# Animesh005/Torus-FHE

Measured on AMD Instinct MI355X. Metric: bootstrapped gates/sec (NAND, N=1024), higher is better.
Workload: dtype f64

## Files before the change

torus-fhe_amd/csrc/thfhe_sk.hip:

```cpp
#include <hip/hip_runtime.h>

#include <algorithm>
#include <cstdlib>
#include <memory>
#include <mutex>
#include <new>
#include <string>
#include <vector>

#include "../../include/thfhe_hip.h"
#include "thfhe_common.h"
#include "thfhe_dag.h"
#include "thfhe_devctx.h"
#include "thfhe_keyswitch.h"
#include "thfhe_lane.h"
#include "thfhe_pack.h"

using namespace thfhe;

namespace {

#include "thfhe_transform.h"

struct Lin {
    int32_t cb, cx, cy;
    int ysel;
};
__host__ __device__ inline bool gate_lin(int op, int which, Lin &L) {
    const int32_t E8 = 1 << 29, E4 = 1 << 30;
    switch (op) {
    case THFHE_NAND: L = Lin{E8, -1, -1, 1}; return true;
    case THFHE_OR: L = Lin{E8, 1, 1, 1}; return true;
    case THFHE_AND: L = Lin{-E8, 1, 1, 1}; return true;
    case THFHE_XOR: L = Lin{E4, 2, 2, 1}; return true;
    case THFHE_XNOR: L = Lin{-E4, -2, -2, 1}; return true;
    case THFHE_NOR: L = Lin{-E8, -1, -1, 1}; return true;
    case THFHE_ANDNY: L = Lin{-E8, -1, 1, 1}; return true;
    case THFHE_ANDYN: L = Lin{-E8, 1, -1, 1}; return true;
    case THFHE_ORNY: L = Lin{E8, -1, 1, 1}; return true;
    case THFHE_ORYN: L = Lin{E8, 1, -1, 1}; return true;
    case THFHE_MUX: L = which == 0 ? Lin{-E8, 1, 1, 1} : Lin{-E8, -1, 1, 2}; return true;
    case kOpIdentity: L = Lin{0, 1, 0, 1}; return true;
    default: return false;
    }
}

__global__ __launch_bounds__(256) void sk_prologue_kernel(const int32_t *__restrict__ in0, const int32_t *__restrict__ in1,
                                                           const int32_t *__restrict__ in2, int op, const int32_t *__restrict__ ops,
                                                           int rot_per_gate, int n, int n_pad, int log2_2n, long jobs,
                                                           int32_t *__restrict__ bara, int32_t *__restrict__ barb) {
    const long job = blockIdx.y;
    const int i = blockIdx.x * 256 + threadIdx.x;
    if (job >= jobs || i > n) return;
    const long gate = job / rot_per_gate;
    const int which = (int)(job % rot_per_gate);
    Lin L;
    gate_lin(ops ? ops[gate] : op, which, L);
    const size_t off = (size_t)gate * (n + 1) + i;
    uint32_t v = (uint32_t)L.cx * (uint32_t)in0[off];
    if (L.cy != 0) v += (uint32_t)L.cy * (uint32_t)(L.ysel == 2 ? in2[off] : in1[off]);
    if (i == n) {
        v += (uint32_t)L.cb;
        barb[job] = modswitch2n((int32_t)v, log2_2n);
    } else {
        bara[job * n_pad + i] = modswitch2n((int32_t)v, log2_2n);
    }
}

THFHE_STAMP_STORAGE

struct BRArgs {
    const cplx *bk;
    const cplx *tw;
    const int32_t *bara;
    const int32_t *barb;
    int32_t *out;
    long jobs;
    int n, n_pad, Bgbit;
    int32_t mu;
    const int32_t *tv;
    const int32_t *lut_idx;
    int theta;
    const int32_t *tv_a;
    const int32_t *mv_w;
    int mv_p, mv_box;
};

constexpr int kGate = 0, kLut = 1, kLutEnc = 2, kLutMv = 3;

#ifndef THFHE_RING_NF
#define THFHE_RING_NF 16
#endif
#ifndef THFHE_RING_LEAN_ROOTS
#define THFHE_RING_LEAN_ROOTS 1
#endif
#ifndef THFHE_RING_READ_FIRST
#define THFHE_RING_READ_FIRST 0
#endif
template <int L, int V = 5, int W = 8, int LUT = kGate>
__global__ __launch_bounds__(64 * W, W == 8 ? 2 : 1) void sk_blind_rotate_ring_kernel(BRArgs a) {
    __shared__ __attribute__((aligned(4096))) int32_t sAcc[W][2048];
    __shared__ cplx sX[W][kXbufSlots];
    __shared__ cplx sRing[3][512];
    constexpr int ROWS = 2 * L;
    constexpr int DPC = 8 / W;
    const int wave = __builtin_amdgcn_readfirstlane(threadIdx.x >> 6);
    const int lane = threadIdx.x & 63;
    const W64 w64{a.tw[TwRing1k::T2 + 1 * 8 + (lane & 7)]};
    const LaneRoots roots{a.tw[TwRing1k::ROOTS + 2 * lane], a.tw[TwRing1k::ROOTS + 2 * lane + 1]};
    const LaneTw tw = make_lane_tw(roots);
    LaneRootsF rootsf{a.tw[TwRing1k::ROOTSF + 2 * lane], a.tw[TwRing1k::ROOTSF + 2 * lane + 1]};
    W64 w64f = w64;
    LaneRoots rootsi = roots;
    const long job = (long)blockIdx.x * W + wave;
    const bool has_job = job < a.jobs;
    int32_t *acc = sAcc[wave];
    cplx *xb = sX[wave];
    const uniform_i32_ptr bara = as_uniform(a.bara + (has_job ? job : 0) * a.n_pad);
    const int Bgbit = a.Bgbit;
    if (has_job) {
        if constexpr (LUT == kLutEnc) {
            const size_t t = a.lut_idx ? (size_t)a.lut_idx[job] * 1024 : 0;
            acc_init_tlwe16(lane, acc, acc + 1024, a.barb[job], a.tv_a + t, a.tv + t);
        } else if constexpr (LUT == kLutMv) acc_init_tv16(lane, acc, acc + 1024, a.barb[job], a.tv);
        else if constexpr (LUT) acc_init_tv16(lane, acc, acc + 1024, a.barb[job], a.tv + (a.lut_idx ? (size_t)a.lut_idx[job] * 1024 : 0));
        else acc_init16(lane, acc, acc + 1024, a.barb[job], a.mu);
    }

    const long total_chunks = (long)a.n * ROWS * 4;
    const cplx *gsrc = a.bk + wave * (64 * DPC) + lane;
    long q_issue = 0;
    int slot_issue = 0;
    const uint32_t ring_base = (uint32_t)(size_t)(__attribute__((address_space(3))) void *)&sRing[0][0] + (uint32_t)wave * (1024u * DPC);
    auto issue = [&]() {
#pragma unroll
        for (int d = 0; d < DPC; d++) ring_dma(gsrc + 64 * d, ring_base + (uint32_t)slot_issue * 8192u + 1024u * d);
        if (q_issue + 1 < total_chunks) {
            gsrc += 512;
            q_issue++;
        }
        slot_issue = slot_issue == 2 ? 0 : slot_issue + 1;
    };
    __syncthreads();
    issue();
    issue();
    issue();
    int slot_use = 0;
    STAMP_DECL;

    for (int i = 0; i < a.n; i++) {
        const int ai = bara[i];
        const bool active = has_job && ai != 0;
        const int a2n = ai & 2047;
        cplx S[2][2][8];
#pragma unroll
        for (int c = 0; c < 2; c++)
#pragma unroll
            for (int h = 0; h < 2; h++)
#pragma unroll
                for (int m = 0; m < 8; m++) S[c][h][m] = cplx{0.0, 0.0};
        constexpr int NF = THFHE_RING_NF;
        uint32_t fld[NF];
#pragma unroll
        for (int r = 0; r < ROWS; r++) {
            cplx z[8];
            if (active) {
                int a2n_r = a2n;
                asm volatile("" : "+s"(a2n_r));
                if (r % L == 0) rotated_fields_keep<NF, W == 4>(lane, acc + (r / L) * 1024, a2n_r, L, Bgbit, fld);
                asm volatile("" : "+s"(a2n_r));
                mixed_digits_z<NF>(lane, acc + (r / L) * 1024, a2n_r, (r % L) + 1, L, Bgbit, fld, z);
                if (V & 4) {
                    if (THFHE_RING_LEAN_ROOTS && W == 8) opaque_in_place(rootsf.s), opaque_in_place(rootsf.w);
                    wave_fft_fwd_f(lane, z, xb, rootsf);
                } else if (!(V & 1)) wave_fft_fwd_r(lane, z, xb, roots, w64);
                else if (THFHE_RING_LEAN_ROOTS && W == 8) wave_fft_fwd_q(lane, z, xb, LaneRoots{opaque_cplx(roots.b), opaque_cplx(roots.s)}, w64);
                else wave_fft_fwd_q(lane, z, xb, tw, w64);
            }
            STAMP(0);
            cplx bA[4], bB[4];
#pragma unroll
            for (int c4 = 0; c4 < 4; c4++) {
                if (c4 == 0) ring_barrier<2 * DPC>(); else ring_barrier<DPC>();
                STAMP(1);
                const cplx *B = &sRing[slot_use][0];
#if THFHE_RING_READ_FIRST
                if (active) {
#pragma unroll
                    for (int m = 0; m < 4; m++) bA[m] = B[m * 64 + lane];
                }
                __builtin_amdgcn_sched_barrier(0);
                if (c4 > 0) issue();
                if (active) {
#else
                if (c4 > 0) issue();
                if (active) {
#pragma unroll
                    for (int m = 0; m < 4; m++) bA[m] = B[m * 64 + lane];
#endif
                    if (c4 > 0) {
#pragma unroll
                        for (int m = 0; m < 4; m++) cfma(S[(c4 - 1) >> 1][(c4 - 1) & 1][4 + m], z[4 + m], bB[m]);
                    }
#pragma unroll
                    for (int m = 0; m < 4; m++) bB[m] = B[(4 + m) * 64 + lane];
#pragma unroll
                    for (int m = 0; m < 4; m++) cfma(S[c4 >> 1][c4 & 1][m], z[m], bA[m]);
                }
                slot_use = slot_use == 2 ? 0 : slot_use + 1;
                STAMP(2);
            }
            ring_barrier<2 * DPC>();
            issue();
            STAMP(1);
            if (active) {
#pragma unroll
                for (int m = 0; m < 4; m++) cfma(S[1][1][4 + m], z[4 + m], bB[m]);
            }
            STAMP(2);
        }
        if (active) {
            wave_sync();
            cplx bc[4];
            if (V & 4) {
                if (THFHE_RING_LEAN_ROOTS && W == 8) opaque_in_place(rootsi.b);
                make_untwist_f(rootsi.b, bc);
            }
#pragma unroll
            for (int c = 0; c < 2; c++) {
                if (V & 4) {
                    wave_fft_inv_f<THFHE_RING_LEAN_ROOTS && W == 8>(lane, S[c][0], xb, w64f, rootsi, bc);
                    wave_fft_inv_f<THFHE_RING_LEAN_ROOTS && W == 8>(lane, S[c][1], xb, w64f, rootsi, bc);
                } else if ((V & 1) && !(V & 2)) {
                    if (THFHE_RING_LEAN_ROOTS && W == 8) {
                        wave_fft_inv_q(lane, S[c][0], xb, LaneRoots{opaque_cplx(roots.b), opaque_cplx(roots.s)}, w64);
                        wave_fft_inv_q(lane, S[c][1], xb, LaneRoots{opaque_cplx(roots.b), opaque_cplx(roots.s)}, w64);
                    } else {
                        wave_fft_inv_q(lane, S[c][0], xb, tw, w64);
                        wave_fft_inv_q(lane, S[c][1], xb, tw, w64);
                    }
                } else {
                    wave_fft_inv_r(lane, S[c][0], xb, roots, w64);
                    wave_fft_inv_r(lane, S[c][1], xb, roots, w64);
                }
                acc_update16(lane, acc + c * 1024, S[c][0], S[c][1]);
            }
            wave_sync();
        }
        STAMP(3);
    }
    STAMP_FLUSH(blockIdx.x, wave);
    asm volatile("s_waitcnt vmcnt(0)" ::: "memory");
    if (has_job) {
        if constexpr (LUT == kLutMv) {
            const uniform_i32_ptr w = as_uniform(a.mv_w) + (size_t)(a.lut_idx ? as_uniform(a.lut_idx)[job] : 0) * a.theta * a.mv_p;
            for (int j = 0; j < a.theta; j++) extract_mv16(lane, acc, acc + 1024, w + j * a.mv_p, a.mv_p, a.mv_box, a.out + (job * a.theta + j) * 1025);
        } else if constexpr (LUT) {
            for (int j = 0; j < a.theta; j++) extract_at16(lane, acc, acc + 1024, j, a.out + (job * a.theta + j) * 1025);
        } else {
            extract16(lane, acc, acc + 1024, a.out + job * 1025);
        }
    }
}

__device__ __forceinline__ void wg_barrier() { asm volatile("s_waitcnt lgkmcnt(0)\n\ts_barrier" ::: "memory"); }
__device__ __forceinline__ void pin() { asm volatile("" ::: "memory"); }

template <int L, int PACE = 1, int LUT = kGate>
__global__ __launch_bounds__(512, 2) void sk_blind_rotate_coop_kernel(BRArgs a) {
    constexpr int ROWS = 2 * L;
    __shared__ __attribute__((aligned(4096))) int32_t sAcc[2048];
    __shared__ cplx sSpec[ROWS][512];
    __shared__ cplx sX[8][kXbufSlots];
    const int wave = __builtin_amdgcn_readfirstlane(threadIdx.x >> 6);
    const int lane = threadIdx.x & 63;
    const W64 w64{a.tw[TwRing1k::T2 + 1 * 8 + (lane & 7)]};
    const LaneRoots roots{a.tw[TwRing1k::ROOTS + 2 * lane], a.tw[TwRing1k::ROOTS + 2 * lane + 1]};
    const long job = blockIdx.x;
    const uniform_i32_ptr bara = as_uniform(a.bara + job * a.n_pad);
    const int Bgbit = a.Bgbit;
    if (wave == 0) {
        if constexpr (LUT == kLutEnc) {
            const size_t t = a.lut_idx ? (size_t)a.lut_idx[job] * 1024 : 0;
            acc_init_tlwe16(lane, sAcc, sAcc + 1024, a.barb[job], a.tv_a + t, a.tv + t);
        } else if constexpr (LUT == kLutMv) acc_init_tv16(lane, sAcc, sAcc + 1024, a.barb[job], a.tv);
        else if constexpr (LUT) acc_init_tv16(lane, sAcc, sAcc + 1024, a.barb[job], a.tv + (a.lut_idx ? (size_t)a.lut_idx[job] * 1024 : 0));
        else acc_init16(lane, sAcc, sAcc + 1024, a.barb[job], a.mu);
    }
    const int c = (wave >> 1) & 1, h = wave & 1, half = wave >> 2, r0 = half * L;
    unsigned int *ap = reinterpret_cast<unsigned int *>(sAcc) + c * 1024;
    cplx *xb = sX[wave];

    int i = 0;
    while (i < a.n && bara[i] == 0) i++;
    cplx B[L][8];
    if (i < a.n) {
#pragma unroll
        for (int r = 0; r < L; r++) load8(lane, B[r], a.bk + bk_spec_index(i, r0 + r, c, h, ROWS));
    }
    wg_barrier();
    STAMP_DECL;
    while (i < a.n) {
        const int a2n = bara[i] & 2047;
        int inext = i + 1;
        while (inext < a.n && bara[inext] == 0) inext++;
        const int inl = inext < a.n ? inext : i;
        if (wave < ROWS) {
            cplx z[8];
            rotated_digits_z(lane, sAcc + (wave / L) * 1024, a2n, (wave % L) + 1, L, Bgbit, z);
            wave_fft_fwd_q(lane, z, xb, roots, w64);
#pragma unroll
            for (int m = 0; m < 8; m++) sSpec[wave][m * 64 + lane] = z[m];
        }
        STAMP(0);
        wg_barrier();
        STAMP(1);
        cplx S[8];
#pragma unroll
        for (int m = 0; m < 8; m++) S[m] = cplx{0.0, 0.0};
#pragma unroll
        for (int r = 0; r < L; r++) {
            cplx z[8];
#pragma unroll
            for (int m = 0; m < 8; m++) z[m] = sSpec[r0 + r][m * 64 + lane];
            mac8r(S, z, B[r]);
            pin();
        }
        STAMP(2);
        if (half == 1) {
#pragma unroll
            for (int m = 0; m < 8; m++) xb[m * 64 + lane] = S[m];
            pin();
            STAMP(3);
            wg_barrier();
            STAMP(4);
#pragma unroll
            for (int r = 0; r < L; r++) {
                const cplx *src = a.bk + bk_spec_index(inl, r0 + r, c, h, ROWS);
#pragma unroll
                for (int m = 0; m < 8; m++) {
                    B[r][m] = src[m * 64 + lane];
                    pin();
                    __builtin_amdgcn_s_sleep(PACE);
                }
            }
        } else {
            load8(lane, B[0], a.bk + bk_spec_index(inl, r0, c, h, ROWS));
            pin();
            STAMP(3);
            wg_barrier();
            STAMP(4);
            const cplx *px = sX[wave + 4];
#pragma unroll
            for (int m = 0; m < 8; m++) {
                const cplx v = px[m * 64 + lane];
                S[m].re += v.re;
                S[m].im += v.im;
            }
            wave_sync();
            invr_seg1(lane, S, xb, w64);
            pin();
            if (L > 1) load8(lane, B[L > 1 ? 1 : 0], a.bk + bk_spec_index(inl, r0 + 1, c, h, ROWS));
            pin();
            wave_sync();
            inv_seg2_ld(lane, S, xb);
            dft8<-1>(S);
            pin();
            if (L > 2) load8(lane, B[L > 2 ? 2 : 0], a.bk + bk_spec_index(inl, r0 + 2, c, h, ROWS));
            if (L > 3) load8(lane, B[L > 3 ? 3 : 0], a.bk + bk_spec_index(inl, r0 + 3, c, h, ROWS));
            pin();
            wave_transpose_hi3(S);
            invq_seg3(S, roots);
#pragma unroll
            for (int m = 0; m < 8; m++) {
                const int q = lane + 64 * m;
                atomicAdd(ap + q, round_lo32(S[m].re) << (16 * h));
                atomicAdd(ap + q + 512, round_lo32(S[m].im) << (16 * h));
            }
        }
        STAMP(3);
        wg_barrier();
        STAMP(5);
        i = inext;
    }
    STAMP_FLUSH(blockIdx.x, wave);
    if constexpr (LUT == kLutMv) {
        const uniform_i32_ptr w = as_uniform(a.mv_w) + (size_t)(a.lut_idx ? as_uniform(a.lut_idx)[job] : 0) * a.theta * a.mv_p;
        for (int j = wave; j < a.theta; j += 8)
            extract_mv16(lane, sAcc, sAcc + 1024, w + j * a.mv_p, a.mv_p, a.mv_box, a.out + (job * a.theta + j) * 1025);
    } else if constexpr (LUT) {
        if (wave < a.theta) extract_at16(lane, sAcc, sAcc + 1024, wave, a.out + (job * a.theta + wave) * 1025);
    } else {
        if (wave == 0) extract16(lane, sAcc, sAcc + 1024, a.out + job * 1025);
    }
}

__global__ __launch_bounds__(256) void sk_linear_kernel(const int32_t *__restrict__ in0, int32_t *__restrict__ out, size_t words, int negate) {
    const size_t q = (size_t)blockIdx.x * 256 + threadIdx.x;
    if (q < words) out[q] = negate ? (int32_t)(0u - (uint32_t)in0[q]) : in0[q];
}

}

struct THFHE_INTERNAL thfhe_ctx : DevCtx {
    thfhe_params p;
    int rec_words() const { return p.n + 1; }
    DevBuf d_bk;
    KsKey ksk;
    int coop_max_jobs = 768;
    int ring4_max_jobs = 1024;
    int n_pad = 0;
    DevBuf d_bara, d_barb, d_u;
    DevBuf d_tv, d_lut_idx;
    DevBuf d_tva;
    DevBuf d_mv_w;
    DevBuf d_tree_tab, d_tree_lwe, d_tree_a, d_tree_b;
    DevBuf d_dag_enc_a, d_dag_enc_b, d_dag_tv1;
    DevBuf d_dag_mv_tv0, d_dag_mv_w;
    DevBuf d_dag_lhe_tab_a, d_dag_lhe_tab_b, d_dag_lhe_fin_a, d_dag_lhe_fin_b, d_dag_lhe_words;
    DevBuf d_lhe_a, d_lhe_b, d_lhe_in[4];
    DevBuf d_wfa_tab;
    DevBuf d_sc_tab, d_sc_idx;
    int cus = 0;
    int wfa_chunk = 0;
    size_t tree_slice = 65536;
    Stage stage;
    DagBuffers dag;
    size_t dag_slice = 28672;
    hipEvent_t grp_ev[2] = {nullptr, nullptr};
    bool grp_valid = false;
    ~thfhe_ctx() {
        for (hipEvent_t e : grp_ev)
            if (e) (void)hipEventDestroy(e);
    }
};

struct THFHE_INTERNAL thfhe_tgsw_set {
    thfhe_ctx *ctx = nullptr;
    DevBuf spec;
    size_t count = 0;
    int d = 0;
};

namespace {

constexpr int kMaxEncLuts = 1 << 18;

int ensure_workspace(thfhe_ctx *c, size_t jobs) {
    int rc = c->d_bara.grow(jobs * c->n_pad * sizeof(int32_t));
    if (!rc) rc = c->d_barb.grow(jobs * sizeof(int32_t));
    if (!rc) rc = c->d_u.grow(jobs * 1025 * sizeof(int32_t));
    return rc;
}

template <int L, int LUT>
void launch_coop(const BRArgs &a, hipStream_t s) {
#ifdef THFHE_VARIANTS
    static const int pace = std::getenv("THFHE_COOP_PACE") ? std::atoi(std::getenv("THFHE_COOP_PACE")) : 1;
    if (!LUT && pace == 0) { hipLaunchKernelGGL((sk_blind_rotate_coop_kernel<L, 0>), dim3((unsigned)a.jobs), dim3(512), 0, s, a); return; }
    if (!LUT && pace == 2) { hipLaunchKernelGGL((sk_blind_rotate_coop_kernel<L, 2>), dim3((unsigned)a.jobs), dim3(512), 0, s, a); return; }
    if (!LUT && pace == 4) { hipLaunchKernelGGL((sk_blind_rotate_coop_kernel<L, 4>), dim3((unsigned)a.jobs), dim3(512), 0, s, a); return; }
#endif
    hipLaunchKernelGGL((sk_blind_rotate_coop_kernel<L, 1, LUT>), dim3((unsigned)a.jobs), dim3(512), 0, s, a);
}
template <int L, int LUT>
void launch_ring4(const BRArgs &a, hipStream_t s) {
    hipLaunchKernelGGL((sk_blind_rotate_ring_kernel<L, 5, 4, LUT>), dim3((unsigned)((a.jobs + 3) / 4)), dim3(256), 0, s, a);
}
template <int L, int LUT>
void launch_ring8(const BRArgs &a, hipStream_t s) {
    const dim3 grid((unsigned)((a.jobs + 7) / 8)), block(512);
#ifdef THFHE_VARIANTS
    static const int variant = std::getenv("THFHE_RING_VARIANT") ? std::atoi(std::getenv("THFHE_RING_VARIANT")) : 0;
    if (!LUT && variant == 8) { hipLaunchKernelGGL((sk_blind_rotate_ring_kernel<L, 0>), grid, block, 0, s, a); return; }
    if (!LUT && variant == 1) { hipLaunchKernelGGL((sk_blind_rotate_ring_kernel<L, 1>), grid, block, 0, s, a); return; }
    if (!LUT && variant == 3) { hipLaunchKernelGGL((sk_blind_rotate_ring_kernel<L, 3>), grid, block, 0, s, a); return; }
#endif
    hipLaunchKernelGGL((sk_blind_rotate_ring_kernel<L, 5, 8, LUT>), grid, block, 0, s, a);
}

template <int L, int LUT>
void launch_br(const BRArgs &a, hipStream_t s, int coop_max, int ring4_max) {
    auto piece = [&](long first, long count) {
        BRArgs b = a;
        b.bara += first * a.n_pad, b.barb += first, b.jobs = count;
        b.out += first * (LUT ? a.theta : 1) * 1025;
        if (LUT && b.lut_idx) b.lut_idx += first;
        return b;
    };
    constexpr long kRound = 2048;
    const long full = (coop_max > 0 || ring4_max > 0) ? a.jobs / kRound * kRound : a.jobs;
    if (full > 0) launch_ring8<L, LUT>(piece(0, full), s);
    const long r = a.jobs - full;
    if (r == 0) return;
    if (r <= coop_max) launch_coop<L, LUT>(piece(full, r), s);
    else if (r <= ring4_max) launch_ring4<L, LUT>(piece(full, r), s);
    else if (ring4_max > 0 && coop_max > 0 && r <= ring4_max + (coop_max < 256 ? coop_max : 256)) {
        launch_ring4<L, LUT>(piece(full, ring4_max), s);
        launch_coop<L, LUT>(piece(full + ring4_max, r - ring4_max), s);
    } else launch_ring8<L, LUT>(piece(full, r), s);
}

template <int LUT>
int launch_rotations(thfhe_ctx *c, const BRArgs &a) {
    switch (c->p.l) {
    case 1: launch_br<1, LUT>(a, c->stream, c->coop_max_jobs, c->ring4_max_jobs); break;
    case 2: launch_br<2, LUT>(a, c->stream, c->coop_max_jobs, c->ring4_max_jobs); break;
    case 3: launch_br<3, LUT>(a, c->stream, c->coop_max_jobs, c->ring4_max_jobs); break;
    case 4: launch_br<4, LUT>(a, c->stream, c->coop_max_jobs, c->ring4_max_jobs); break;
    default: return thfhe_fail(THFHE_E_UNSUPPORTED, "decomposition length l must be 1..4");
    }
    return THFHE_OK;
}

int enqueue_rotations(thfhe_ctx *c, int op, const int32_t *d0, const int32_t *d1, const int32_t *d2, size_t gates,
                      int rot_per_gate, int32_t mu, const int32_t *d_ops = nullptr) {
// ... 736 lines not shown
```

Baseline: 139,800.

## Restructure bootstrap-key ring prefetch to borrow FFT scratch as fourth slot

```diff
diff --git a/torus-fhe_amd/csrc/thfhe_ring_schedule.h b/torus-fhe_amd/csrc/thfhe_ring_schedule.h
--- /dev/null
+++ b/torus-fhe_amd/csrc/thfhe_ring_schedule.h
@@ -0,0 +1,69 @@
+#pragma once
+
+namespace thfhe {
+namespace ring_schedule {
+
+constexpr int kChunksPerRow = 4;
+constexpr int kResidentSlots = 3;
+constexpr int kBorrowedSlot = 3;
+constexpr int kSlots = 4;
+constexpr int kSlotBytes = 8192;
+constexpr int kSliceBytes = 1024;
+
+enum Barrier : int { kBarA = 0, kBarX = 1, kBarB = 2, kBarriersPerRow = 3 };
+
+struct ChunkPlan {
+    int slot;
+    int issue_barrier;
+    int issue_row;
+    int certify_barrier;
+    int free_barrier;
+};
+constexpr ChunkPlan kPlan[kChunksPerRow] = {
+    {0, kBarX, -1, kBarA, kBarX},
+    {1, kBarX, -1, kBarA, kBarX},
+    {2, kBarX, -1, kBarA, kBarX},
+    {kBorrowedSlot, kBarA, 0, kBarX, kBarB},
+};
+constexpr int kPrologueIssues = 3;
+
+constexpr int first_consumed(int b) {
+    int c = 0;
+    while (c < kChunksPerRow && kPlan[c].certify_barrier < b) c++;
+    return c;
+}
+constexpr int issues_at(int b) {
+    int k = 0;
+    for (int c = 0; c < kChunksPerRow; c++) k += kPlan[c].issue_barrier == b;
+    return k;
+}
+constexpr int issue_chunk(int b, int k) {
+    for (int row = 0; row >= -1; row--)
+        for (int c = 0; c < kChunksPerRow; c++)
+            if (kPlan[c].issue_barrier == b && kPlan[c].issue_row == row && k-- == 0) return c;
+    return -1;
+}
+constexpr int issue_slot(int b, int k) { return kPlan[issue_chunk(b, k)].slot; }
+constexpr int vmcnt_at(int b) {
+    int younger = 0;
+    for (int back = 0; back < kBarriersPerRow; back++) {
+        const int bb = (b - 1 - back + 2 * kBarriersPerRow) % kBarriersPerRow;
+        const bool prev_row = b - 1 - back < 0;
+        for (int k = issues_at(bb) - 1; k >= 0; k--) {
+            const int c = issue_chunk(bb, k);
+            const int rows_ahead = (kPlan[c].issue_row == -1 ? 1 : 0) - (prev_row ? 1 : 0);
+            if (rows_ahead == 0 && kPlan[c].certify_barrier <= b) return younger;
+            younger++;
+        }
+    }
+    return younger;
+}
+
+static_assert(first_consumed(kBarA) == 0 && first_consumed(kBarX) == 3 && first_consumed(kBarB) == 4 && first_consumed(kBarriersPerRow) == 4, "");
+static_assert(issues_at(kBarA) == 1 && issues_at(kBarX) == 3 && issues_at(kBarB) == 0, "");
+static_assert(issue_chunk(kBarA, 0) == 3 && issue_chunk(kBarX, 0) == 0 && issue_chunk(kBarX, 1) == 1 && issue_chunk(kBarX, 2) == 2, "");
+static_assert(vmcnt_at(kBarA) == 0 && vmcnt_at(kBarX) == 0 && vmcnt_at(kBarB) == 3, "");
+static_assert(issues_at(kBarA) + issues_at(kBarX) + issues_at(kBarB) == kChunksPerRow, "");
+
+}
+}
diff --git a/torus-fhe_amd/csrc/thfhe_sk.hip b/torus-fhe_amd/csrc/thfhe_sk.hip
--- a/torus-fhe_amd/csrc/thfhe_sk.hip
+++ b/torus-fhe_amd/csrc/thfhe_sk.hip
@@ -15,6 +15,7 @@
 #include "thfhe_keyswitch.h"
 #include "thfhe_lane.h"
 #include "thfhe_pack.h"
+#include "thfhe_ring_schedule.h"
 
 using namespace thfhe;
 
@@ -94,9 +95,6 @@
 #ifndef THFHE_RING_LEAN_ROOTS
 #define THFHE_RING_LEAN_ROOTS 1
 #endif
-#ifndef THFHE_RING_READ_FIRST
-#define THFHE_RING_READ_FIRST 0
-#endif
 template <int L, int V = 5, int W = 8, int LUT = kGate>
 __global__ __launch_bounds__(64 * W, W == 8 ? 2 : 1) void sk_blind_rotate_ring_kernel(BRArgs a) {
     __shared__ __attribute__((aligned(4096))) int32_t sAcc[W][2048];
@@ -104,6 +102,7 @@
     __shared__ cplx sRing[3][512];
     constexpr int ROWS = 2 * L;
     constexpr int DPC = 8 / W;
+    namespace RS = ring_schedule;
     const int wave = __builtin_amdgcn_readfirstlane(threadIdx.x >> 6);
     const int lane = threadIdx.x & 63;
     const W64 w64{a.tw[TwRing1k::T2 + 1 * 8 + (lane & 7)]};
@@ -127,25 +126,25 @@
         else acc_init16(lane, acc, acc + 1024, a.barb[job], a.mu);
     }
 
-    const long total_chunks = (long)a.n * ROWS * 4;
+    const long total_chunks = (long)a.n * ROWS * RS::kChunksPerRow;
     const cplx *gsrc = a.bk + wave * (64 * DPC) + lane;
     long q_issue = 0;
-    int slot_issue = 0;
+    static_assert(RS::kResidentSlots * RS::kSlotBytes == sizeof(sRing) && RS::kSlotBytes <= sizeof(sX[0]), "ring schedule against the LDS layout");
     const uint32_t ring_base = (uint32_t)(size_t)(__attribute__((address_space(3))) void *)&sRing[0][0] + (uint32_t)wave * (1024u * DPC);
-    auto issue = [&]() {
-#pragma unroll
-        for (int d = 0; d < DPC; d++) ring_dma(gsrc + 64 * d, ring_base + (uint32_t)slot_issue * 8192u + 1024u * d);
+    const uint32_t lent_base = (uint32_t)(size_t)(__attribute__((address_space(3))) void *)&sX[0][0] + (uint32_t)wave * (1024u * DPC);
+    auto issue = [&](int slot) {
+        const uint32_t dst = slot == RS::kBorrowedSlot ? lent_base : ring_base + (uint32_t)slot * (uint32_t)RS::kSlotBytes;
+#pragma unroll
+        for (int d = 0; d < DPC; d++) ring_dma(gsrc + 64 * d, dst + 1024u * d);
         if (q_issue + 1 < total_chunks) {
             gsrc += 512;
             q_issue++;
         }
-        slot_issue = slot_issue == 2 ? 0 : slot_issue + 1;
     };
+    auto slot_ptr = [&](int slot) -> const cplx * { return slot == RS::kBorrowedSlot ? &sX[0][0] : &sRing[slot][0]; };
     __syncthreads();
-    issue();
-    issue();
-    issue();
-    int slot_use = 0;
+#pragma unroll
+    for (int k = 0; k < RS::kPrologueIssues; k++) issue(RS::kPlan[k].slot);
     STAMP_DECL;
 
     for (int i = 0; i < a.n; i++) {
@@ -179,25 +178,11 @@
             }
             STAMP(0);
             cplx bA[4], bB[4];
-#pragma unroll
-            for (int c4 = 0; c4 < 4; c4++) {
-                if (c4 == 0) ring_barrier<2 * DPC>(); else ring_barrier<DPC>();
-                STAMP(1);
-                const cplx *B = &sRing[slot_use][0];
-#if THFHE_RING_READ_FIRST
+            auto consume = [&](int c4) {
+                const cplx *B = slot_ptr(RS::kPlan[c4].slot);
                 if (active) {
 #pragma unroll
                     for (int m = 0; m < 4; m++) bA[m] = B[m * 64 + lane];
-                }
-                __builtin_amdgcn_sched_barrier(0);
-                if (c4 > 0) issue();
-                if (active) {
-#else
-                if (c4 > 0) issue();
-                if (active) {
-#pragma unroll
-                    for (int m = 0; m < 4; m++) bA[m] = B[m * 64 + lane];
-#endif
                     if (c4 > 0) {
 #pragma unroll
                         for (int m = 0; m < 4; m++) cfma(S[(c4 - 1) >> 1][(c4 - 1) & 1][4 + m], z[4 + m], bB[m]);
@@ -207,11 +192,23 @@
 #pragma unroll
                     for (int m = 0; m < 4; m++) cfma(S[c4 >> 1][c4 & 1][m], z[m], bA[m]);
                 }
-                slot_use = slot_use == 2 ? 0 : slot_use + 1;
-                STAMP(2);
-            }
-            ring_barrier<2 * DPC>();
-            issue();
+            };
+            ring_barrier<RS::vmcnt_at(RS::kBarA) * DPC>();
+            STAMP(1);
+#pragma unroll
+            for (int k = 0; k < RS::issues_at(RS::kBarA); k++) issue(RS::issue_slot(RS::kBarA, k));
+#pragma unroll
+            for (int c4 = RS::first_consumed(RS::kBarA); c4 < RS::first_consumed(RS::kBarX); c4++) consume(c4);
+            STAMP(2);
+            ring_barrier<RS::vmcnt_at(RS::kBarX) * DPC>();
+            STAMP(1);
+#pragma unroll
+            for (int k = 0; k < RS::issues_at(RS::kBarX); k++) issue(RS::issue_slot(RS::kBarX, k));
+#pragma unroll
+            for (int c4 = RS::first_consumed(RS::kBarX); c4 < RS::first_consumed(RS::kBarB); c4++) consume(c4);
+            STAMP(2);
+            ring_barrier<RS::vmcnt_at(RS::kBarB) * DPC>();
+            static_assert(RS::issues_at(RS::kBarB) == 0 && RS::first_consumed(RS::kBarB) == RS::kChunksPerRow, "nothing is issued or read after barrier B");
             STAMP(1);
             if (active) {
 #pragma unroll
```

Measured after the change: 142,500, median of 6. 1.9% higher.
